# player4771/YOLO-DBL

Hardware: AMD Instinct MI355X
Metric: images/sec @640×640 bs=32 (1/2/4/8 GPU) + mAP@0.5 vs CPU ref (higher is better)
Workload: dtype fp16; 1 GPU; YOLO-DBL-n 640x640 bs=32/GPU fp16 forward+decode+NMS (conf .25, iou .7, max_det 300); model=yolov13n_DBL, global_batch=32, imgsz=640, nc=3, parallelism=dp1, streams_per_gpu=2

## Files before the change

include/ydbl.h:

```cpp
#ifndef YDBL_H
#define YDBL_H

#include <stdint.h>

#ifdef __cplusplus
extern "C" {
#endif

enum { YDBL_OK = 0, YDBL_EINVAL = 1, YDBL_ELAUNCH = 2, YDBL_ECAPACITY = 3 };
enum { YDBL_F32 = 0, YDBL_F16 = 1 };
enum { YDBL_ACT_NONE = 0, YDBL_ACT_SILU = 1, YDBL_ACT_GELU = 2, YDBL_ACT_SIGMOID = 3 };
enum { YDBL_RES_NONE = 0, YDBL_RES_ADD = 1, YDBL_RES_MUL = 2 };

typedef struct {
  void* ptr;
  int32_t n, h, w, c;
  int32_t cs;
  int32_t dtype;
} ydbl_view;

typedef struct {
  ydbl_view x, y, r;
  const void* w;
  const float* bias;
  int32_t kh, kw, stride, pad, dil;
  int32_t kpad;
  int32_t act, res_mode;
  ydbl_view y2, r2;
  float a2, b2;
  const float* dq;
  float qscale;
  void* workspace;
  int64_t workspace_bytes;
} ydbl_conv_desc;
int ydbl_conv2d_nhwc(const ydbl_conv_desc* d, void* stream);
int64_t ydbl_conv_workspace(const ydbl_conv_desc* d);

typedef struct {
  ydbl_view x, y, r;
  const float* dw_w;
  const void* pw_w;
  const float* bias;
  int32_t k, stride, pad, dil;
  int32_t kpad, act, res_mode;
  const float* dw_bias;
  int32_t dw_act;
  const float* tail_w;
  const float* tail_b;
  ydbl_view tail_y;
  int32_t tail_n;
  float* cand_box;
  float* cand_score;
  int32_t* cand_cls;
  int32_t* cand_idx;
  int32_t* cand_count;
  int32_t cand_cap;
  float conf_thres;
  int32_t multi_label;
  int32_t nclasses;
  const int32_t* classes;
  float level_stride;
  int32_t anchor0;
  ydbl_view box;
  int32_t zero_counts;
  int32_t y_unused;
  uint8_t* tile_mask;
  int32_t mask_tiles_x;
  int32_t mask_tiles_img;
  uint8_t* mask_zero;
  int32_t mask_zero_bytes;
} ydbl_dsconv_desc;
int ydbl_dsconv_nhwc(const ydbl_dsconv_desc* d, void* stream);

typedef struct {
  ydbl_view x, y, r;
  const float* w;
  const float* bias;
  int32_t kh, kw, stride, pad, dil;
  int32_t act, res_mode;
} ydbl_dwconv_desc;
int ydbl_dwconv2d_nhwc(const ydbl_dwconv_desc* d, void* stream);

int ydbl_dwconv2d_pair_nhwc(const ydbl_dwconv_desc* d0, const ydbl_dwconv_desc* d1, void* stream);

typedef struct {
  const float* const* x;
  const float* amax;
} ydbl_input_bind;

int32_t ydbl_batch_max_work_ints(void);
void ydbl_batch_max_work_init(int32_t* host_work);
int ydbl_batch_max(const float* x, int64_t n, int32_t* work, float* amax, float* scale, void* stream);
int ydbl_batch_max_bound(const float* const* xword, int64_t n, int32_t* work, float* amax, float* scale,
                         void* stream);

int ydbl_input_nchw_to_nhwc(const float* x, int32_t n, int32_t c, int32_t h, int32_t w, float scale,
                            const ydbl_view* y, const ydbl_input_bind* bind, void* stream);

int ydbl_conv_stem(const float* x, int32_t n, int32_t cin, int32_t h, int32_t w, float scale, const float* wt,
                   const float* bias, int32_t k, int32_t stride, int32_t act, const ydbl_view* y,
                   const ydbl_input_bind* bind, void* stream);

int ydbl_gate_add(const ydbl_view* a, const ydbl_view* b, float gate, const ydbl_view* y, void* stream);

int ydbl_channel_gate_add(const ydbl_view* a, const ydbl_view* b, const float* gate, const ydbl_view* y,
                          void* stream);

typedef struct {
  ydbl_view qkv, y, v;
  int32_t heads, area;
  float scale;
} ydbl_area_attn_desc;
int ydbl_area_attn(const ydbl_area_attn_desc* d, void* stream);

int ydbl_pool_up_concat(const ydbl_view* p_lo, const ydbl_view* p_mid, const ydbl_view* p_hi,
                        const ydbl_view* y, void* stream);

int ydbl_dysample(const ydbl_view* x, const ydbl_view* off, int32_t groups, const ydbl_view* y, void* stream);
typedef struct {
  ydbl_view x, off;
  int32_t groups;
  ydbl_view y, y2, r2;
  float a2, b2;
} ydbl_dysample_desc;
int ydbl_dysample_ex(const ydbl_dysample_desc* d, void* stream);
typedef struct {
  ydbl_view x;
  const void* off_w;
  const float* off_b;
  int32_t groups;
  ydbl_view y, y2, r2;
  float a2, b2;
} ydbl_dysample2_desc;
int ydbl_dysample2(const ydbl_dysample2_desc* d, void* stream);

int ydbl_lsk_gate(const ydbl_view* attn, const float* sw, const float* sb, const ydbl_view* out,
                  void* workspace, void* stream);
int64_t ydbl_lsk_gate_workspace(int32_t n, int32_t h, int32_t w);
typedef struct {
  ydbl_view x, a1, a2, attn, y;
  const void* w12;
  const float* b12;
  const float* sw;
  const float* sb;
  const void* w;
  const float* b;
  float* agg;
} ydbl_lsk_desc;
int ydbl_lsk_attn(const ydbl_lsk_desc* d, void* stream);
int ydbl_lsk_out(const ydbl_lsk_desc* d, void* stream);

typedef struct {
  ydbl_view x;
  ydbl_view xp;
  ydbl_view y;
  int32_t num_edges, num_heads;
  const float* proto_base;
  const float* ctx_w;
  const float* ctx_b;
  const float* edge_w;
  const float* edge_b;
  const float* node_w;
  const float* node_b;
  void* workspace;
  const void* pre_w;
  const float* pre_b;
} ydbl_hg_desc;
int64_t ydbl_hg_workspace(int32_t n, int32_t tokens, int32_t dim, int32_t edges);
int ydbl_hg_context(const ydbl_hg_desc* d, void* stream);
int ydbl_hg_propagate(const ydbl_hg_desc* d, void* stream);
int64_t ydbl_hg_fused_workspace(int32_t n, int32_t tokens, int32_t dim, int32_t edges, int32_t dtype);
int ydbl_hg_fused(const ydbl_hg_desc* d, void* stream);
int ydbl_hg_fused_pair(const ydbl_hg_desc* d0, const ydbl_hg_desc* d1, void* stream);

typedef struct {
  ydbl_view box[3], cls[3];
  int32_t nl, nc;
  float stride[3];
  float conf_thres;
  int32_t multi_label;
  const int32_t* classes; int32_t nclasses;
  float* y_ref;
  float* cand_box;
  float* cand_score;
  int32_t* cand_cls;
  int32_t* cand_idx;
  int32_t* cand_count;
  int32_t cap;
} ydbl_decode_desc;
int ydbl_detect_decode(const ydbl_decode_desc* d, void* stream);

typedef struct {
  float scale;
  float flip_w;
  int32_t a_lo, a_hi;
  int32_t pos_base;
  int32_t y_stride;
  int32_t append;
} ydbl_decode_aug;
int ydbl_detect_decode_aug(const ydbl_decode_desc* d, const ydbl_decode_aug* g, void* stream);

typedef struct {
  const float* pred;
  int32_t n, nc, A;
  float conf_thres;
  int32_t multi_label;
  const int32_t* classes; int32_t nclasses;
  float* cand_box; float* cand_score; int32_t* cand_cls; int32_t* cand_idx; int32_t* cand_count;
  int32_t cap;
} ydbl_pred_cand_desc;
int ydbl_pred_candidates(const ydbl_pred_cand_desc* d, void* stream);

typedef struct {
  const float* cand_box; const float* cand_score; const int32_t* cand_cls; const int32_t* cand_idx;
  const int32_t* cand_count;
  int32_t n, cap;
  double iou_thres;
  int32_t max_det, max_nms, agnostic;
  float max_wh;
  float clip_w, clip_h;
  float* out; int32_t* out_count;
  void* workspace;
  int64_t out_stride, count_stride;
  int32_t per_image;
} ydbl_nms_desc;
int64_t ydbl_nms_workspace(int32_t n, int32_t cap, int32_t max_nms);
int ydbl_nms(const ydbl_nms_desc* d, void* stream);

typedef struct {
  const float* x;
  int32_t n, cin, h, w;
  float scale;
  int32_t c0;
  const void* params;
  ydbl_view y;
  ydbl_input_bind bind;
// ... 163 lines not shown
```

yolo-dbl_amd/csrc/misc.hip:

```cpp
#include "common.hpp"

namespace ydbl {

template <typename T>
__global__ __launch_bounds__(256) void dwconv_kernel(DView<const T> x, DView<T> y, DView<const T> r,
                                                     const float* __restrict__ w, const float* __restrict__ bias,
                                                     int KH, int KW, int S, int PAD, int DIL, int act) {
  constexpr int V = Vec<T>::N;
  const int cg = y.c / V;
  const int64_t idx = (int64_t)blockIdx.x * blockDim.x + threadIdx.x;
  const int64_t total = (int64_t)y.n * y.h * y.w * cg;
  if (idx >= total) return;
  const int c0 = (int)(idx % cg) * V;
  int64_t pix = idx / cg;
  const int ox = (int)(pix % y.w);
  const int64_t t = pix / y.w;
  const int oy = (int)(t % y.h);
  const int b = (int)(t / y.h);
  float acc[V];
#pragma unroll
  for (int q = 0; q < V; ++q) acc[q] = 0.f;
  for (int ky = 0; ky < KH; ++ky) {
    const int iy = oy * S - PAD + ky * DIL;
    if (iy < 0 || iy >= x.h) continue;
// ... 331 lines not shown
    for (int q = 0; q < V; ++q) s[q] += v[q];
    load_f<V>(lo.at(b, 2 * oy + 1, 2 * ox) + c, v);
#pragma unroll
    for (int q = 0; q < V; ++q) s[q] += v[q];
    load_f<V>(lo.at(b, 2 * oy + 1, 2 * ox + 1) + c, v);
#pragma unroll
    for (int q = 0; q < V; ++q) o[q] = (s[q] + v[q]) / 4.0f;
  } else if (c < clo + cmid) {
    load_f<V>(mid.at(b, oy, ox) + (c - clo), o);
  } else {
    load_f<V>(hi.at(b, oy >> 1, ox >> 1) + (c - clo - cmid), o);
  }
  store_f<V>(y.at(b, oy, ox) + c, o);
}

template <typename T>
__global__ __launch_bounds__(256) void dysample_kernel(DView<const T> x, DView<const T> off, int G, DView<T> y,
                                                       DView<T> y2, DView<const T> r2, float a2, float b2) {
  constexpr int V = Vec<T>::N;
  const int cpg = x.c / G;
  const int cgv = cpg / V;
  const int64_t idx = (int64_t)blockIdx.x * blockDim.x + threadIdx.x;
  const int64_t total = (int64_t)y.n * y.h * y.w * G * cgv;
  if (idx >= total) return;
  const int cv = (int)(idx % cgv);
  int64_t t = idx / cgv;
  const int gi = (int)(t % G);
  t /= G;
  const int ox2 = (int)(t % y.w);
  t /= y.w;
  const int oy2 = (int)(t % y.h);
  const int b = (int)(t / y.h);
  const int H = x.h, W = x.w;
  const int h = oy2 >> 1, w = ox2 >> 1, si = oy2 & 1, sj = ox2 & 1;
  const T* op = off.at(b, h, w);
  const float offx = float(op[gi * 4 + si * 2 + sj]);
  const float offy = float(op[4 * G + gi * 4 + si * 2 + sj]);
  const float gx = 2.0f * ((float(w) + 0.5f) + offx) / float(W) - 1.0f;
  const float gy = 2.0f * ((float(h) + 0.5f) + offy) / float(H) - 1.0f;
  float ix = ((gx + 1.0f) * float(W) - 1.0f) / 2.0f;
  float iy = ((gy + 1.0f) * float(H) - 1.0f) / 2.0f;
  ix = fminf(float(W - 1), fmaxf(ix, 0.0f));
  iy = fminf(float(H - 1), fmaxf(iy, 0.0f));
  const int x0 = (int)floorf(ix), y0 = (int)floorf(iy);
  const int x1 = x0 + 1, y1 = y0 + 1;
  const float wnw = (float(x1) - ix) * (float(y1) - iy);
  const float wne = (ix - float(x0)) * (float(y1) - iy);
  const float wsw = (float(x1) - ix) * (iy - float(y0));
  const float wse = (ix - float(x0)) * (iy - float(y0));
  const int c0 = gi * cpg + cv * V;
  const bool xin = x1 < W, yin = y1 < H;
  const int x1c = xin ? x1 : x0, y1c = yin ? y1 : y0;
  float vnw[V], vne[V], vsw[V], vse[V];
  load_f<V>(x.at(b, y0, x0) + c0, vnw);
  load_f<V>(x.at(b, y0, x1c) + c0, vne);
  load_f<V>(x.at(b, y1c, x0) + c0, vsw);
  load_f<V>(x.at(b, y1c, x1c) + c0, vse);
  const float kne = xin ? wne : 0.f, ksw = yin ? wsw : 0.f, kse = xin && yin ? wse : 0.f;
  float acc[V];
#pragma unroll
  for (int q = 0; q < V; ++q) {
    acc[q] = blend4(vnw[q], wnw, vne[q], kne, vsw[q], ksw, vse[q], kse);
  }
  store_f<V>(y.at(b, oy2, ox2) + c0, acc);
  if (y2.p) {
    float rv[V], o2[V];
    load_f<V>(r2.at(b, oy2, ox2) + c0, rv);
#pragma unroll
    for (int q = 0; q < V; ++q) o2[q] = pad_mix(a2, round_to<T>(acc[q]), b2, rv[q]);
    store_f<V>(y2.at(b, oy2, ox2) + c0, o2);
  }
}

template <typename T>
__global__ __launch_bounds__(256) void lsk_stats_kernel(DView<const T> attn, float* __restrict__ agg) {
  constexpr int V = Vec<T>::N, L = 32;
  const int64_t t = (int64_t)blockIdx.x * blockDim.x + threadIdx.x;
  const int64_t pix = t / L;
  const int sub = (int)(t % L);
  const bool live = pix < (int64_t)attn.n * attn.h * attn.w;
  const T* p = attn.pix(live ? pix : 0);
  float s = 0.f, m = -INFINITY;
  for (int c = sub * V; c < attn.c; c += L * V) {
    float v[V];
    load_f<V>(p + c, v);
#pragma unroll
    for (int q = 0; q < V; ++q) {
      s += v[q];
      m = fmaxf(m, v[q]);
    }
  }
#pragma unroll
  for (int o = L / 2; o > 0; o >>= 1) {
    s += __shfl_xor(s, o);
    m = fmaxf(m, __shfl_xor(m, o));
  }
  if (live && sub == 0) {
    agg[pix * 2 + 0] = s / float(attn.c);
    agg[pix * 2 + 1] = m;
  }
}

template <typename T>
__global__ __launch_bounds__(256) void lsk_gate_kernel(DView<const T> attn, const float* __restrict__ agg,
                                                       const float* __restrict__ sw, const float* __restrict__ sb,
                                                       DView<T> out) {
  constexpr int V = Vec<T>::N;
  const int half = out.c;
  const int cg = half / V;
  const int64_t idx = (int64_t)blockIdx.x * blockDim.x + threadIdx.x;
  if (idx >= (int64_t)out.n * out.h * out.w * cg) return;
  const int c0 = (int)(idx % cg) * V;
  const int64_t pix = idx / cg;
  const int ox = (int)(pix % out.w);
  const int64_t t = pix / out.w;
  const int oy = (int)(t % out.h);
  const int b = (int)(t / out.h);
  const bool split = cg % 16 == 0;
  const int t0 = split ? (int)(idx & 15) : 0, ts = split ? 16 : 1;
  float s0 = 0.f, s1 = 0.f;
  for (int tap = t0; tap < 98; tap += ts) {
    const int ci = tap / 49, ky = (tap % 49) / 7, kx = tap % 7;
    const int iy = oy - 3 + ky, ix = ox - 3 + kx;
    if (iy < 0 || iy >= out.h || ix < 0 || ix >= out.w) continue;
    const float a = agg[(((int64_t)b * out.h + iy) * out.w + ix) * 2 + ci];
    s0 = fmaf(sw[((0 * 2 + ci) * 7 + ky) * 7 + kx], a, s0);
    s1 = fmaf(sw[((1 * 2 + ci) * 7 + ky) * 7 + kx], a, s1);
  }
  if (split) {
#pragma unroll
    for (int o = 8; o > 0; o >>= 1) {
      s0 += __shfl_xor(s0, o);
      s1 += __shfl_xor(s1, o);
    }
  }
  s0 = sigmoidf_(s0 + sb[0]);
  s1 = sigmoidf_(s1 + sb[1]);
  float a1[V], a2[V], o[V];
  load_f<V>(attn.pix(pix) + c0, a1);
  load_f<V>(attn.pix(pix) + half + c0, a2);
#pragma unroll
  for (int q = 0; q < V; ++q) o[q] = gate_mix(a1[q], s0, a2[q], s1);
  store_f<V>(out.pix(pix) + c0, o);
}

template <typename T>
static DView<const T> cview(const ydbl_view* v) {
  if (!v) return DView<const T>{nullptr, 0, 0, 0, 0, 0};
  return DView<const T>{reinterpret_cast<const T*>(v->ptr), v->n, v->h, v->w, v->c, v->cs};
}

static unsigned nblk(int64_t n) { return (unsigned)cdiv(n, 256); }

}

using namespace ydbl;

extern "C" int ydbl_dwconv2d_nhwc(const ydbl_dwconv_desc* d, void* stream) {
  if (!d) return fail(YDBL_EINVAL, "dwconv: null descriptor");
  if (check_view(&d->x, "dwconv.x", true) || check_view(&d->y, "dwconv.y", true)) return YDBL_EINVAL;
  if (d->x.c != d->y.c || d->x.n != d->y.n || d->x.dtype != d->y.dtype) return fail(YDBL_EINVAL, "dwconv: x/y mismatch");
  const int ho = (d->x.h + 2 * d->pad - d->dil * (d->kh - 1) - 1) / d->stride + 1;
  const int wo = (d->x.w + 2 * d->pad - d->dil * (d->kw - 1) - 1) / d->stride + 1;
  if (ho != d->y.h || wo != d->y.w) return fail(YDBL_EINVAL, "dwconv: output spatial size mismatch");
  if (!d->w) return fail(YDBL_EINVAL, "dwconv: null weights");
  const bool res = d->res_mode == YDBL_RES_ADD;
  if (d->res_mode != YDBL_RES_NONE && !res) return fail(YDBL_EINVAL, "dwconv: only residual ADD is supported");
  if (res && (check_view(&d->r, "dwconv.r", true) || d->r.c != d->y.c || d->r.n != d->y.n || d->r.h != d->y.h ||
              d->r.w != d->y.w || d->r.dtype != d->y.dtype))
    return fail(YDBL_EINVAL, "dwconv: residual shape mismatch");
  hipStream_t s = as_stream(stream);
  const int V = d->x.dtype == YDBL_F16 ? 8 : 4;
  const int64_t total = (int64_t)d->y.n * d->y.h * d->y.w * (d->y.c / V);
  if (d->kh == d->kw) {
    const bool done = d->x.dtype == YDBL_F16
                          ? launch_dw_lds<_Float16>(d, cview<_Float16>(&d->x), dview<_Float16>(d->y),
                                                   cview<_Float16>(res ? &d->r : nullptr), s)
                          : launch_dw_lds<float>(d, cview<float>(&d->x), dview<float>(d->y),
                                                cview<float>(res ? &d->r : nullptr), s);
    if (done) return check_launch("ydbl_dwconv2d_nhwc");
  }
  if (d->x.dtype == YDBL_F16)
    dwconv_kernel<_Float16><<<nblk(total), 256, 0, s>>>(cview<_Float16>(&d->x), dview<_Float16>(d->y),
                                                        cview<_Float16>(res ? &d->r : nullptr), d->w, d->bias,
                                                        d->kh, d->kw, d->stride, d->pad, d->dil, epi_act(d->act));
  else
    dwconv_kernel<float><<<nblk(total), 256, 0, s>>>(cview<float>(&d->x), dview<float>(d->y),
                                                     cview<float>(res ? &d->r : nullptr), d->w, d->bias, d->kh, d->kw,
                                                     d->stride, d->pad, d->dil, epi_act(d->act));
  return check_launch("ydbl_dwconv2d_nhwc");
}

extern "C" int ydbl_dwconv2d_pair_nhwc(const ydbl_dwconv_desc* d0, const ydbl_dwconv_desc* d1, void* stream) {
  if (!d0 || !d1) return fail(YDBL_EINVAL, "dw_pair: null descriptor");
  if (d1->x.ptr != d0->y.ptr || d1->x.cs != d0->y.cs || d1->x.c != d0->y.c)
    return fail(YDBL_EINVAL, "dw_pair: d1.x must be d0.y");
  const bool pair = d0->kh == 5 && d0->kw == 5 && d0->dil == 1 && d1->kh == 7 && d1->kw == 7 && d1->dil == 3 &&
                    d0->stride == 1 && d1->stride == 1 && d0->res_mode == YDBL_RES_NONE &&
                    d1->res_mode == YDBL_RES_NONE && d0->x.h == d0->y.h && d0->x.w == d0->y.w &&
                    d1->y.h == d0->y.h && d1->y.w == d0->y.w && d0->x.h * d0->x.w <= DWP_HWMAX &&
                    d0->x.dtype == d0->y.dtype && d1->y.dtype == d0->y.dtype && d0->x.c == d0->y.c &&
                    d1->y.c == d0->y.c && d0->x.n == d0->y.n && d1->y.n == d0->y.n;
  const int V = d0->x.dtype == YDBL_F16 ? 8 : 4;
  constexpr int CV = 2;
  if (!pair || d0->y.c % (CV * V) || !d0->w || !d1->w || check_view(&d0->x, "dw_pair.x", true) ||
      check_view(&d0->y, "dw_pair.y0", true) || check_view(&d1->y, "dw_pair.y1", true)) {
    const int r = ydbl_dwconv2d_nhwc(d0, stream);
    return r ? r : ydbl_dwconv2d_nhwc(d1, stream);
  }
  hipStream_t s = as_stream(stream);
  const unsigned blocks = (unsigned)(d0->y.n * (d0->y.c / (CV * V)));
  constexpr int NT = 1024;
  if (d0->x.dtype == YDBL_F16)
    dw_pair_kernel<_Float16, 5, 1, 7, 3, CV, NT><<<blocks, NT, 0, s>>>(
        cview<_Float16>(&d0->x), dview<_Float16>(d0->y), dview<_Float16>(d1->y), d0->w, d0->bias, d1->w, d1->bias,
        d0->pad, d1->pad, epi_act(d0->act), epi_act(d1->act));
  else
    dw_pair_kernel<float, 5, 1, 7, 3, CV, NT><<<blocks, NT, 0, s>>>(
        cview<float>(&d0->x), dview<float>(d0->y), dview<float>(d1->y), d0->w, d0->bias, d1->w, d1->bias, d0->pad,
        d1->pad, epi_act(d0->act), epi_act(d1->act));
  return check_launch("ydbl_dwconv2d_pair_nhwc");
}

extern "C" int ydbl_input_nchw_to_nhwc(const float* x, int32_t n, int32_t c, int32_t h, int32_t w, float scale,
                                       const ydbl_view* y, const ydbl_input_bind* bind, void* stream) {
  if (!x) return fail(YDBL_EINVAL, "input: null x");
  if (check_view(y, "input.y", true)) return YDBL_EINVAL;
  if (y->n != n || y->h != h || y->w != w || y->c < c) return fail(YDBL_EINVAL, "input: shape mismatch");
  hipStream_t s = as_stream(stream);
  const int64_t total = (int64_t)n * h * w;
  if (y->dtype == YDBL_F16)
    input_kernel<_Float16><<<nblk(total), 256, 0, s>>>(x, n, c, h, w, scale, dview<_Float16>(*y), input_bind(bind));
  else
    input_kernel<float><<<nblk(total), 256, 0, s>>>(x, n, c, h, w, scale, dview<float>(*y), input_bind(bind));
  return check_launch("ydbl_input_nchw_to_nhwc");
}

extern "C" int ydbl_gate_add(const ydbl_view* a, const ydbl_view* b, float gate, const ydbl_view* y, void* stream) {
  if (check_view(a, "gate.a", true) || check_view(b, "gate.b", true) || check_view(y, "gate.y", true)) return YDBL_EINVAL;
  if (a->c != y->c || b->c != y->c || a->n * a->h * a->w != y->n * y->h * y->w ||
      b->n * b->h * b->w != y->n * y->h * y->w || a->dtype != y->dtype || b->dtype != y->dtype)
    return fail(YDBL_EINVAL, "gate_add: shape mismatch");
  hipStream_t s = as_stream(stream);
  const int V = y->dtype == YDBL_F16 ? 8 : 4;
  const int64_t total = (int64_t)y->n * y->h * y->w * (y->c / V);
  if (y->dtype == YDBL_F16)
    gate_add_kernel<_Float16><<<nblk(total), 256, 0, s>>>(cview<_Float16>(a), cview<_Float16>(b), gate, dview<_Float16>(*y));
  else
    gate_add_kernel<float><<<nblk(total), 256, 0, s>>>(cview<float>(a), cview<float>(b), gate, dview<float>(*y));
  return check_launch("ydbl_gate_add");
}

extern "C" int ydbl_channel_gate_add(const ydbl_view* a, const ydbl_view* b, const float* gate, const ydbl_view* y,
                                     void* stream) {
  if (check_view(a, "cgate.a", true) || check_view(b, "cgate.b", true) || check_view(y, "cgate.y", true)) return YDBL_EINVAL;
  if (!gate || reinterpret_cast<uintptr_t>(gate) % 16) return fail(YDBL_EINVAL, "channel_gate_add: gate must be a 16-byte aligned fp32 vector");
  if (a->c != y->c || b->c != y->c || a->n * a->h * a->w != y->n * y->h * y->w ||
      b->n * b->h * b->w != y->n * y->h * y->w || a->dtype != y->dtype || b->dtype != y->dtype)
    return fail(YDBL_EINVAL, "channel_gate_add: shape mismatch");
  hipStream_t s = as_stream(stream);
  const int V = y->dtype == YDBL_F16 ? 8 : 4;
  const int64_t total = (int64_t)y->n * y->h * y->w * (y->c / V);
  if (y->dtype == YDBL_F16)
    channel_gate_add_kernel<_Float16><<<nblk(total), 256, 0, s>>>(cview<_Float16>(a), cview<_Float16>(b), gate,
                                                                   dview<_Float16>(*y));
  else
    channel_gate_add_kernel<float><<<nblk(total), 256, 0, s>>>(cview<float>(a), cview<float>(b), gate, dview<float>(*y));
  return check_launch("ydbl_channel_gate_add");
}

extern "C" int ydbl_pool_up_concat(const ydbl_view* lo, const ydbl_view* mid, const ydbl_view* hi, const ydbl_view* y,
                                   void* stream) {
  if (check_view(y, "concat.y", true)) return YDBL_EINVAL;
  int ctot = 0;
  if (lo) {
    if (check_view(lo, "concat.lo", true)) return YDBL_EINVAL;
    if (lo->h != 2 * y->h || lo->w != 2 * y->w || lo->n != y->n) return fail(YDBL_EINVAL, "concat: lo must be 2x output");
    ctot += lo->c;
  }
  if (mid) {
    if (check_view(mid, "concat.mid", true)) return YDBL_EINVAL;
    if (mid->h != y->h || mid->w != y->w || mid->n != y->n) return fail(YDBL_EINVAL, "concat: mid must match output");
    ctot += mid->c;
  }
  if (hi) {
    if (check_view(hi, "concat.hi", true)) return YDBL_EINVAL;
    if (2 * hi->h != y->h || 2 * hi->w != y->w || hi->n != y->n) return fail(YDBL_EINVAL, "concat: hi must be 1/2 output");
    ctot += hi->c;
  }
  if (ctot != y->c) return fail(YDBL_EINVAL, "concat: channel sum mismatch");
  hipStream_t s = as_stream(stream);
  const int V = y->dtype == YDBL_F16 ? 8 : 4;
  const int64_t total = (int64_t)y->n * y->h * y->w * (y->c / V);
  if (y->dtype == YDBL_F16)
    pool_up_concat_kernel<_Float16><<<nblk(total), 256, 0, s>>>(cview<_Float16>(lo), cview<_Float16>(mid),
                                                                 cview<_Float16>(hi), dview<_Float16>(*y));
  else
    pool_up_concat_kernel<float><<<nblk(total), 256, 0, s>>>(cview<float>(lo), cview<float>(mid), cview<float>(hi),
                                                              dview<float>(*y));
  return check_launch("ydbl_pool_up_concat");
}

static int dysample_go(const ydbl_view* x, const ydbl_view* off, int32_t groups, const ydbl_view* y,
                       const ydbl_view* y2, const ydbl_view* r2, float a2, float b2, void* stream) {
  if (check_view(x, "dysample.x", true) || check_view(off, "dysample.off", false) || check_view(y, "dysample.y", true))
    return YDBL_EINVAL;
  const int V = y->dtype == YDBL_F16 ? 8 : 4;
  if (groups < 1 || x->c % groups || (x->c / groups) % V) return fail(YDBL_EINVAL, "dysample: bad groups");
  if (off->c != 8 * groups || off->h != x->h || off->w != x->w || y->h != 2 * x->h || y->w != 2 * x->w ||
      y->c != x->c || off->dtype != x->dtype || y->dtype != x->dtype)
    return fail(YDBL_EINVAL, "dysample: shape mismatch");
  const bool two = y2 && y2->ptr;
  if (two) {
    if (check_view(y2, "dysample.y2", true) || check_view(r2, "dysample.r2", true)) return YDBL_EINVAL;
    auto same = [&](const ydbl_view* v) {
      return v->n == y->n && v->h == y->h && v->w == y->w && v->c == y->c && v->dtype == y->dtype;
    };
    if (!same(y2) || !same(r2)) return fail(YDBL_EINVAL, "dysample: y2/r2 must match y");
  }
  hipStream_t s = as_stream(stream);
  const int64_t total = (int64_t)y->n * y->h * y->w * groups * (x->c / groups / V);
  if (y->dtype == YDBL_F16)
    dysample_kernel<_Float16><<<nblk(total), 256, 0, s>>>(
        cview<_Float16>(x), cview<_Float16>(off), groups, dview<_Float16>(*y),
        two ? dview<_Float16>(*y2) : DView<_Float16>{nullptr, 0, 0, 0, 0, 0}, cview<_Float16>(two ? r2 : nullptr), a2, b2);
  else
    dysample_kernel<float><<<nblk(total), 256, 0, s>>>(
        cview<float>(x), cview<float>(off), groups, dview<float>(*y),
        two ? dview<float>(*y2) : DView<float>{nullptr, 0, 0, 0, 0, 0}, cview<float>(two ? r2 : nullptr), a2, b2);
  return check_launch("ydbl_dysample");
}

extern "C" int ydbl_dysample(const ydbl_view* x, const ydbl_view* off, int32_t groups, const ydbl_view* y,
                             void* stream) {
  return dysample_go(x, off, groups, y, nullptr, nullptr, 0.f, 0.f, stream);
}

extern "C" int ydbl_dysample_ex(const ydbl_dysample_desc* d, void* stream) {
  if (!d) return fail(YDBL_EINVAL, "dysample: null descriptor");
  return dysample_go(&d->x, &d->off, d->groups, &d->y, &d->y2, &d->r2, d->a2, d->b2, stream);
}

extern "C" int64_t ydbl_lsk_gate_workspace(int32_t n, int32_t h, int32_t w) { return (int64_t)n * h * w * 2 * 4; }

extern "C" int ydbl_lsk_gate(const ydbl_view* attn, const float* sw, const float* sb, const ydbl_view* out,
                             void* workspace, void* stream) {
  if (check_view(attn, "lsk.attn", true) || check_view(out, "lsk.out", true)) return YDBL_EINVAL;
  if (attn->c != 2 * out->c || attn->n != out->n || attn->h != out->h || attn->w != out->w ||
      attn->dtype != out->dtype)
    return fail(YDBL_EINVAL, "lsk: shape mismatch");
  if (!sw || !sb || !workspace) return fail(YDBL_EINVAL, "lsk: null weights/workspace");
  hipStream_t s = as_stream(stream);
  float* agg = reinterpret_cast<float*>(workspace);
  const int64_t npix = (int64_t)out->n * out->h * out->w;
  const int V = out->dtype == YDBL_F16 ? 8 : 4;
  if (out->dtype == YDBL_F16) {
    lsk_stats_kernel<_Float16><<<nblk(npix * 32), 256, 0, s>>>(cview<_Float16>(attn), agg);
    lsk_gate_kernel<_Float16><<<nblk(npix * (out->c / V)), 256, 0, s>>>(cview<_Float16>(attn), agg, sw, sb,
                                                                         dview<_Float16>(*out));
  } else {
    lsk_stats_kernel<float><<<nblk(npix * 32), 256, 0, s>>>(cview<float>(attn), agg);
    lsk_gate_kernel<float><<<nblk(npix * (out->c / V)), 256, 0, s>>>(cview<float>(attn), agg, sw, sb,
                                                                      dview<float>(*out));
// ... 4 lines not shown
```

yolo-dbl_amd/ydbl/_lib.py:

```python

from __future__ import annotations

import ctypes as C
import os
from pathlib import Path

import torch

LIB_PATH = Path(os.environ.get("YDBL_LIB", Path(__file__).resolve().parent / "libydbl.so"))

F32, F16 = 0, 1
ACT_NONE, ACT_SILU, ACT_GELU, ACT_SIGMOID = 0, 1, 2, 3
RES_NONE, RES_ADD, RES_MUL = 0, 1, 2


class View(C.Structure):
    _fields_ = [("ptr", C.c_void_p), ("n", C.c_int32), ("h", C.c_int32), ("w", C.c_int32), ("c", C.c_int32),
                ("cs", C.c_int32), ("dtype", C.c_int32)]


class ConvDesc(C.Structure):
    _fields_ = [("x", View), ("y", View), ("r", View), ("w", C.c_void_p), ("bias", C.c_void_p),
                ("kh", C.c_int32), ("kw", C.c_int32), ("stride", C.c_int32), ("pad", C.c_int32), ("dil", C.c_int32),
                ("kpad", C.c_int32), ("act", C.c_int32), ("res_mode", C.c_int32),
# ... 20 lines not shown
                ("zero_counts", C.c_int32), ("y_unused", C.c_int32),
                ("tile_mask", C.c_void_p), ("mask_tiles_x", C.c_int32), ("mask_tiles_img", C.c_int32),
                ("mask_zero", C.c_void_p), ("mask_zero_bytes", C.c_int32)]
    g2_w = g0_w = None


class HgDesc(C.Structure):
    _fields_ = [("x", View), ("xp", View), ("y", View), ("num_edges", C.c_int32), ("num_heads", C.c_int32),
                ("proto_base", C.c_void_p), ("ctx_w", C.c_void_p), ("ctx_b", C.c_void_p),
                ("edge_w", C.c_void_p), ("edge_b", C.c_void_p), ("node_w", C.c_void_p), ("node_b", C.c_void_p),
                ("workspace", C.c_void_p), ("pre_w", C.c_void_p), ("pre_b", C.c_void_p)]


class DecodeDesc(C.Structure):
    _fields_ = [("box", View * 3), ("cls", View * 3), ("nl", C.c_int32), ("nc", C.c_int32),
                ("stride", C.c_float * 3), ("conf_thres", C.c_float), ("multi_label", C.c_int32),
                ("classes", C.c_void_p), ("nclasses", C.c_int32), ("y_ref", C.c_void_p),
                ("cand_box", C.c_void_p), ("cand_score", C.c_void_p), ("cand_cls", C.c_void_p),
                ("cand_idx", C.c_void_p), ("cand_count", C.c_void_p), ("cap", C.c_int32)]


class DecodeAug(C.Structure):
    _fields_ = [("scale", C.c_float), ("flip_w", C.c_float), ("a_lo", C.c_int32), ("a_hi", C.c_int32),
                ("pos_base", C.c_int32), ("y_stride", C.c_int32), ("append", C.c_int32)]


class ScaleImgDesc(C.Structure):
    _fields_ = [("x", C.c_void_p), ("n", C.c_int32), ("c", C.c_int32), ("h", C.c_int32), ("w", C.c_int32),
                ("sh", C.c_int32), ("sw", C.c_int32), ("hp", C.c_int32), ("wp", C.c_int32), ("flip", C.c_int32),
                ("pad_value", C.c_float), ("y", C.c_void_p)]


class PredCandDesc(C.Structure):
    _fields_ = [("pred", C.c_void_p), ("n", C.c_int32), ("nc", C.c_int32), ("A", C.c_int32),
                ("conf_thres", C.c_float), ("multi_label", C.c_int32), ("classes", C.c_void_p),
                ("nclasses", C.c_int32), ("cand_box", C.c_void_p), ("cand_score", C.c_void_p),
                ("cand_cls", C.c_void_p), ("cand_idx", C.c_void_p), ("cand_count", C.c_void_p), ("cap", C.c_int32)]


class NmsDesc(C.Structure):
    _fields_ = [("cand_box", C.c_void_p), ("cand_score", C.c_void_p), ("cand_cls", C.c_void_p),
                ("cand_idx", C.c_void_p), ("cand_count", C.c_void_p), ("n", C.c_int32), ("cap", C.c_int32),
                ("iou_thres", C.c_double), ("max_det", C.c_int32), ("max_nms", C.c_int32), ("agnostic", C.c_int32),
                ("max_wh", C.c_float), ("clip_w", C.c_float), ("clip_h", C.c_float), ("out", C.c_void_p),
                ("out_count", C.c_void_p), ("workspace", C.c_void_p), ("out_stride", C.c_int64),
                ("count_stride", C.c_int64), ("per_image", C.c_int32)]


class InputBind(C.Structure):
    _fields_ = [("x", C.c_void_p), ("amax", C.c_void_p)]


class Stem2Desc(C.Structure):
    _fields_ = [("x", C.c_void_p), ("n", C.c_int32), ("cin", C.c_int32), ("h", C.c_int32), ("w", C.c_int32),
                ("scale", C.c_float), ("c0", C.c_int32), ("params", C.c_void_p), ("y", View), ("bind", InputBind)]


class DySampleDesc(C.Structure):
    _fields_ = [("x", View), ("off", View), ("groups", C.c_int32), ("y", View), ("y2", View), ("r2", View),
                ("a2", C.c_float), ("b2", C.c_float)]


class DySample2Desc(C.Structure):
    _fields_ = [("x", View), ("off_w", C.c_void_p), ("off_b", C.c_void_p), ("groups", C.c_int32), ("y", View),
                ("y2", View), ("r2", View), ("a2", C.c_float), ("b2", C.c_float)]


class LskDesc(C.Structure):
    _fields_ = [("x", View), ("a1", View), ("a2", View), ("attn", View), ("y", View), ("w12", C.c_void_p),
                ("b12", C.c_void_p), ("sw", C.c_void_p), ("sb", C.c_void_p), ("w", C.c_void_p), ("b", C.c_void_p),
                ("agg", C.c_void_p)]


class BottleneckDesc(C.Structure):
    _fields_ = [("x", View), ("y", View), ("c", C.c_int32), ("add", C.c_int32), ("tile_h", C.c_int32),
                ("params", C.c_void_p), ("c_mid", C.c_int32), ("pw", C.c_int32),
                ("tile_mask", C.c_void_p), ("cand_box", C.c_void_p), ("cand_idx", C.c_void_p),
                ("cand_count", C.c_void_p), ("cand_cap", C.c_int32), ("level_stride", C.c_float),
                ("anchor0", C.c_int32), ("nc", C.c_int32), ("multi_label", C.c_int32)]


class LetterboxDesc(C.Structure):
    _fields_ = [("src", C.c_void_p), ("src_off", C.c_void_p), ("meta", C.c_void_p), ("n", C.c_int32),
                ("out_h", C.c_int32), ("out_w", C.c_int32), ("pad_value", C.c_float), ("out", C.c_void_p)]


class MatchDesc(C.Structure):
    _fields_ = [("det", C.c_void_p), ("det_count", C.c_void_p), ("n", C.c_int32), ("max_det", C.c_int32),
                ("gt_box", C.c_void_p), ("gt_cls", C.c_void_p), ("gt_ofs", C.c_void_p), ("n_gt", C.c_int32),
                ("iouv", C.c_void_p), ("n_iou", C.c_int32), ("single_cls", C.c_int32), ("correct", C.c_void_p),
                ("workspace", C.c_void_p)]


class ConfusionDesc(C.Structure):
    _fields_ = [("det", C.c_void_p), ("det_count", C.c_void_p), ("n", C.c_int32), ("max_det", C.c_int32),
                ("gt_box", C.c_void_p), ("gt_cls", C.c_void_p), ("gt_ofs", C.c_void_p), ("n_gt", C.c_int32),
                ("nc", C.c_int32), ("conf", C.c_float), ("iou_thres", C.c_float), ("matrix", C.c_void_p),
                ("invalid", C.c_void_p), ("workspace", C.c_void_p)]


class CocoDesc(C.Structure):
    _fields_ = [("det", C.c_void_p), ("det_count", C.c_void_p), ("n", C.c_int32), ("max_det", C.c_int32),
                ("gt_box", C.c_void_p), ("gt_cls", C.c_void_p), ("gt_ofs", C.c_void_p), ("n_gt", C.c_int32),
                ("single_cls", C.c_int32), ("nc", C.c_int32), ("iou_thrs", C.c_void_p), ("n_iou", C.c_int32),
                ("area_rng", C.c_void_p), ("n_area", C.c_int32), ("max_dets", C.c_int32), ("dt_rank", C.c_void_p),
                ("dt_matched", C.c_void_p), ("dt_ignored", C.c_void_p), ("gt_ignore", C.c_void_p),
                ("invalid", C.c_void_p), ("workspace", C.c_void_p)]


class AreaAttnDesc(C.Structure):
    _fields_ = [("qkv", View), ("y", View), ("v", View), ("heads", C.c_int32), ("area", C.c_int32),
                ("scale", C.c_float)]


class AvgPoolDesc(C.Structure):
    _fields_ = [("x", View), ("y", C.c_void_p), ("y_stride", C.c_int64), ("workspace", C.c_void_p),
                ("workspace_bytes", C.c_int64)]


class TrackDesc(C.Structure):
    _fields_ = [("det", C.c_void_p), ("det_count", C.c_void_p), ("n", C.c_int32), ("max_det", C.c_int32),
                ("det_stride", C.c_int64), ("count_stride", C.c_int64), ("hw", C.c_void_p),
                ("track_high_thresh", C.c_double), ("track_low_thresh", C.c_double),
                ("new_track_thresh", C.c_double), ("match_thresh", C.c_double), ("fuse_score", C.c_int32),
                ("track_buffer", C.c_int32), ("max_time_lost", C.c_int32), ("max_tracks", C.c_int32),
                ("trackers", C.c_int32), ("reset_each", C.c_int32), ("out", C.c_void_p), ("out_count", C.c_void_p),
                ("tracked", C.c_void_p), ("out_idx", C.c_void_p), ("state", C.c_void_p), ("state_bytes", C.c_int64)]


class LossDesc(C.Structure):
    _fields_ = [("box", View * 3), ("cls", View * 3), ("nl", C.c_int32), ("nc", C.c_int32), ("reg_max", C.c_int32),
                ("stride", C.c_float * 3), ("gt", C.c_void_p), ("max_labels", C.c_int32), ("topk", C.c_int32),
                ("gain_box", C.c_float), ("gain_cls", C.c_float), ("gain_dfl", C.c_float),
                ("loss", C.c_void_p), ("target_scores_sum", C.c_void_p), ("per_image", C.c_void_p),
                ("fg", C.c_void_p), ("target_gt_idx", C.c_void_p), ("target_score", C.c_void_p),
                ("workspace", C.c_void_p), ("workspace_bytes", C.c_int64)]


class LossGradDesc(C.Structure):
    _fields_ = [("box", View * 3), ("cls", View * 3), ("nl", C.c_int32), ("nc", C.c_int32), ("reg_max", C.c_int32),
                ("stride", C.c_float * 3), ("gt", C.c_void_p), ("max_labels", C.c_int32),
                ("gain_box", C.c_float), ("gain_cls", C.c_float), ("gain_dfl", C.c_float),
                ("fg", C.c_void_p), ("target_gt_idx", C.c_void_p), ("target_score", C.c_void_p),
                ("target_scores_sum", C.c_void_p), ("grad_scale", C.c_void_p), ("batch_scale", C.c_float),
                ("gbox", View * 3), ("gcls", View * 3)]


_P = C.c_void_p
_VP = C.POINTER(View)
SIGNATURES = {
    "ydbl_conv2d_nhwc": ([C.POINTER(ConvDesc), _P], C.c_int),
    "ydbl_dwconv2d_nhwc": ([C.POINTER(DwConvDesc), _P], C.c_int),
    "ydbl_dwconv2d_pair_nhwc": ([C.POINTER(DwConvDesc), C.POINTER(DwConvDesc), _P], C.c_int),
    "ydbl_dsconv_nhwc": ([C.POINTER(DsConvDesc), _P], C.c_int),
    "ydbl_batch_max_work_ints": ([], C.c_int32),
    "ydbl_batch_max_work_init": ([_P], None),
    "ydbl_batch_max": ([_P, C.c_int64, _P, _P, _P, _P], C.c_int),
    "ydbl_batch_max_bound": ([_P, C.c_int64, _P, _P, _P, _P], C.c_int),
    "ydbl_input_nchw_to_nhwc": ([_P, C.c_int32, C.c_int32, C.c_int32, C.c_int32, C.c_float, _VP,
                                 C.POINTER(InputBind), _P], C.c_int),
    "ydbl_conv_stem": ([_P, C.c_int32, C.c_int32, C.c_int32, C.c_int32, C.c_float, _P, _P, C.c_int32, C.c_int32,
                        C.c_int32, _VP, C.POINTER(InputBind), _P], C.c_int),
    "ydbl_gate_add": ([_VP, _VP, C.c_float, _VP, _P], C.c_int),
    "ydbl_channel_gate_add": ([_VP, _VP, _P, _VP, _P], C.c_int),
    "ydbl_area_attn": ([C.POINTER(AreaAttnDesc), _P], C.c_int),
    "ydbl_pool_up_concat": ([_VP, _VP, _VP, _VP, _P], C.c_int),
    "ydbl_dysample": ([_VP, _VP, C.c_int32, _VP, _P], C.c_int),
    "ydbl_dysample_ex": ([C.POINTER(DySampleDesc), _P], C.c_int),
    "ydbl_lsk_gate": ([_VP, _P, _P, _VP, _P, _P], C.c_int),
    "ydbl_lsk_gate_workspace": ([C.c_int32, C.c_int32, C.c_int32], C.c_int64),
    "ydbl_lsk_attn": ([C.POINTER(LskDesc), _P], C.c_int),
    "ydbl_lsk_out": ([C.POINTER(LskDesc), _P], C.c_int),
    "ydbl_hg_workspace": ([C.c_int32, C.c_int32, C.c_int32, C.c_int32], C.c_int64),
    "ydbl_hg_context": ([C.POINTER(HgDesc), _P], C.c_int),
    "ydbl_hg_propagate": ([C.POINTER(HgDesc), _P], C.c_int),
    "ydbl_hg_fused_workspace": ([C.c_int32, C.c_int32, C.c_int32, C.c_int32, C.c_int32], C.c_int64),
    "ydbl_hg_fused": ([C.POINTER(HgDesc), _P], C.c_int),
    "ydbl_hg_fused_pair": ([C.POINTER(HgDesc), C.POINTER(HgDesc), _P], C.c_int),
    "ydbl_dysample2": ([C.POINTER(DySample2Desc), _P], C.c_int),
    "ydbl_detect_decode": ([C.POINTER(DecodeDesc), _P], C.c_int),
    "ydbl_detect_decode_aug": ([C.POINTER(DecodeDesc), C.POINTER(DecodeAug), _P], C.c_int),
    "ydbl_scale_img": ([C.POINTER(ScaleImgDesc), _P], C.c_int),
    "ydbl_pred_candidates": ([C.POINTER(PredCandDesc), _P], C.c_int),
    "ydbl_nms_workspace": ([C.c_int32, C.c_int32, C.c_int32], C.c_int64),
    "ydbl_conv_workspace": ([C.POINTER(ConvDesc)], C.c_int64),
    "ydbl_nms": ([C.POINTER(NmsDesc), _P], C.c_int),
    "ydbl_conv_stem2_params_size": ([C.c_int32], C.c_int64),
    "ydbl_conv_stem2_pack": ([_P, _P, _P, _P, C.c_int32, _P], C.c_int),
    "ydbl_conv_stem2": ([C.POINTER(Stem2Desc), _P], C.c_int),
    "ydbl_bottleneck_params_size": ([C.c_int32], C.c_int64),
    "ydbl_bottleneck_pack": ([_P, _P, _P, _P, C.c_int32, _P], C.c_int),
    "ydbl_bottleneck_nhwc": ([C.POINTER(BottleneckDesc), _P], C.c_int),
    "ydbl_conv3x3_pair_params_size": ([C.c_int32, C.c_int32], C.c_int64),
    "ydbl_conv3x3_pair_pack": ([_P, _P, _P, _P, C.c_int32, C.c_int32, _P], C.c_int),
    "ydbl_detect_box_params_size": ([C.c_int32, C.c_int32], C.c_int64),
    "ydbl_detect_box_pack": ([_P, _P, _P, _P, _P, _P, C.c_int32, C.c_int32, _P], C.c_int),
    "ydbl_letterbox": ([C.POINTER(LetterboxDesc), _P], C.c_int),
    "ydbl_match_workspace": ([C.c_int32, C.c_int32, C.c_int32, C.c_int32], C.c_int64),
    "ydbl_match_predictions": ([C.POINTER(MatchDesc), _P], C.c_int),
    "ydbl_confusion_workspace": ([C.c_int32, C.c_int32, C.c_int32], C.c_int64),
    "ydbl_confusion_matrix": ([C.POINTER(ConfusionDesc), _P], C.c_int),
    "ydbl_coco_workspace": ([C.c_int32, C.c_int32, C.c_int32, C.c_int32], C.c_int64),
    "ydbl_coco_match": ([C.POINTER(CocoDesc), _P], C.c_int),
    "ydbl_global_avgpool_workspace": ([C.POINTER(AvgPoolDesc)], C.c_int64),
    "ydbl_global_avgpool": ([C.POINTER(AvgPoolDesc), _P], C.c_int),
    "ydbl_bytetrack_state_bytes": ([C.c_int32, C.c_int32], C.c_int64),
    "ydbl_bytetrack_update": ([C.POINTER(TrackDesc), _P], C.c_int),
    "ydbl_detect_loss_workspace": ([C.c_int32, C.c_int32, C.c_int32], C.c_int64),
    "ydbl_detect_loss": ([C.POINTER(LossDesc), _P], C.c_int),
    "ydbl_detect_loss_grad": ([C.POINTER(LossGradDesc), _P], C.c_int),
    "ydbl_last_error": ([], C.c_char_p),
    "ydbl_version": ([], C.c_char_p),
}


def _load():
    if not LIB_PATH.exists():
        raise ImportError(
            f"libydbl.so not found at {LIB_PATH}; build it with `python -c \"import __graft_entry__ as g; g.build()\"` "
            "(the HIP path has no fallback)"
        )
    lib = C.CDLL(str(LIB_PATH))
    for name, (args, res) in SIGNATURES.items():
        fn = getattr(lib, name)
        fn.argtypes = args
        fn.restype = res
    return lib


lib = _load()


class YdblError(RuntimeError):
    pass


def check(rc: int, what: str = ""):
    if rc != 0:
        msg = lib.ydbl_last_error().decode(errors="replace")
        raise YdblError(f"{what or 'ydbl'} failed (code {rc}): {msg}")


def dtype_code(dt: torch.dtype) -> int:
    if dt == torch.float16:
        return F16
    if dt == torch.float32:
        return F32
    raise TypeError(f"unsupported activation dtype {dt}")


def version() -> str:
    return lib.ydbl_version().decode()


def batch_max_work(device) -> "torch.Tensor":
    import torch

    host = torch.empty(int(lib.ydbl_batch_max_work_ints()), dtype=torch.int32)
    lib.ydbl_batch_max_work_init(host.data_ptr())
    return host.to(device)
```

yolo-dbl_amd/ydbl/runtime.py:

```python

from __future__ import annotations

import ctypes as C
import operator
import os
import time
from dataclasses import dataclass, field

import torch

from . import _lib
from ._lib import View, lib


SWITCHES = ("YDBL_DS2_OFF", "YDBL_DS_LEAN", "YDBL_HG_UNFUSED", "YDBL_HALO_NB", "YDBL_HALO_SMALL", "YDBL_VW", "YDBL_WSK_HALF",
            "YDBL_LSK_FUSE", "YDBL_NMS_FAST", "YDBL_NMS_GROUPS", "YDBL_SPLITK", "YDBL_NO_BNECK", "YDBL_NO_BOX3",
            "YDBL_NO_CLS_TAIL", "YDBL_DWPW", "YDBL_NO_PAIR3", "YDBL_NO_FUSE_PAD", "YDBL_NO_MERGE", "YDBL_NO_STEM2",
            "YDBL_EPI_GENERIC", "YDBL_NO_SPARSE_BOX", "YDBL_NO_HG_PAIR")


def ydbl_env() -> tuple:
    get = os.environ.get
    return tuple(get(k) for k in SWITCHES)


_STRUCT_EPOCH = [0]


def _bump_epoch(*_):
    _STRUCT_EPOCH[0] += 1


for _reg in ("register_module_parameter_registration_hook", "register_module_buffer_registration_hook",
             "register_module_module_registration_hook"):
    getattr(torch.nn.modules.module, _reg)(_bump_epoch)
_VERSION = operator.attrgetter("_version")


def weights_signature(module: torch.nn.Module) -> tuple:
    c = module.__dict__.get("_wsig_cache")
    if c is None or c[0] != _STRUCT_EPOCH[0]:
        ts = [t for t in (*module.parameters(), *module.buffers()) if t.is_floating_point()]
        c = (_STRUCT_EPOCH[0], ts, hash(tuple((id(t), t.data_ptr()) for t in ts)))
        module.__dict__["_wsig_cache"] = c
    return c[2], sum(map(_VERSION, c[1]))


def round_up(x: int, m: int) -> int:
    return (x + m - 1) // m * m


class TV:

    __slots__ = ("base", "off", "n", "h", "w", "c", "cs")

    def __init__(self, base: torch.Tensor, off: int, n: int, h: int, w: int, c: int, cs: int):
        self.base, self.off, self.n, self.h, self.w, self.c, self.cs = base, off, n, h, w, c, cs

    @property
    def dtype(self):
        return self.base.dtype

    @property
    def ptr(self) -> int:
        return self.base.data_ptr() + self.off * self.base.element_size()

    @property
    def shape(self):
        return (self.n, self.h, self.w, self.c)

    def cslice(self, c0: int, c: int) -> "TV":
        assert 0 <= c0 and c0 + c <= self.c, (c0, c, self.c)
        return TV(self.base, self.off + c0, self.n, self.h, self.w, c, self.cs)

    def with_hw(self, h: int, w: int) -> "TV":
        assert h * w == self.h * self.w
        return TV(self.base, self.off, self.n, h, w, self.c, self.cs)

    def struct(self) -> View:
        return View(self.ptr, self.n, self.h, self.w, self.c, self.cs, _lib.dtype_code(self.dtype))

    def torch(self) -> torch.Tensor:
        return torch.as_strided(
            self.base, (self.n, self.h, self.w, self.c), (self.h * self.w * self.cs, self.w * self.cs, self.cs, 1),
            self.off,
        )

    def nchw(self) -> torch.Tensor:
        return self.torch().permute(0, 3, 1, 2)


@dataclass
class Step:
    fn: object
    args: tuple
    what: str
    keep: list = field(default_factory=list)


class Plan:

    def __init__(self, device: torch.device, dtype: torch.dtype):
        self.device = torch.device(device)
        self.dtype = dtype
        self.steps: list[Step] = []
        self.buffers: list[torch.Tensor] = []
        self.bytes_allocated = 0
        self._writers: dict = {}
        self.fp8_candidates: list = []
        self.fp8_layers: list = []

    def alloc(self, n: int, h: int, w: int, c: int, dtype: torch.dtype | None = None, cs: int | None = None) -> TV:
        dtype = dtype or self.dtype
        cs = cs or round_up(c, 8)
        t = torch.empty(n * h * w * cs, dtype=dtype, device=self.device)
        self.buffers.append(t)
        self.bytes_allocated += t.numel() * t.element_size()
        return TV(t, 0, n, h, w, c, cs)

    def scratch(self, nbytes: int, zero: bool = False) -> torch.Tensor:
        t = (torch.zeros if zero else torch.empty)(max(int(nbytes), 16), dtype=torch.uint8, device=self.device)
        self.buffers.append(t)
        self.bytes_allocated += t.numel()
        return t

    def splitk_scratch(self, nbytes: int) -> torch.Tensor:
        cur = getattr(self, "_splitk", None)
        if cur is None or cur.numel() < nbytes:
            cur = self._splitk = self.scratch(nbytes)
        return cur

    def const(self, t: torch.Tensor) -> torch.Tensor:
        t = t.detach().to(self.device).contiguous()
        self.buffers.append(t)
        return t

    def launch(self, name: str, *args, what: str = "", keep=()):
        self.steps.append(Step(getattr(lib, name), args, what or name, list(keep)))

    @staticmethod
    def _vkey(v: TV):
        return (v.base.data_ptr(), v.off, v.n, v.h, v.w, v.c, v.cs)

    def note_writer(self, y: TV, desc) -> None:
        self._writers[self._vkey(y)] = (len(self.steps) - 1, desc)

    def writer_of(self, v: TV):
        return self._writers.get(self._vkey(v))

    def made_before(self, v: TV, step: int) -> bool:
        w = self.writer_of(v)
        return w is not None and w[0] < step

    def fuse_second_output(self, writer, y2: TV, r2: TV, a2: float, b2: float) -> TV | None:
        _, d = writer
        if not hasattr(d, "y2") or d.y2.ptr:
            return None
        y = d.y
        for v in (y2, r2):
            if (v.n, v.h, v.w, v.c) != (y.n, y.h, y.w, y.c) or _lib.dtype_code(v.dtype) != y.dtype or v.cs % 4:
                return None
            if isinstance(d, (_lib.DySampleDesc, _lib.DySample2Desc)):
                vec = 16 // v.base.element_size()
                if v.cs % vec or v.c % vec or v.ptr % 16:
                    return None
        d.y2, d.r2, d.a2, d.b2 = y2.struct(), r2.struct(), float(a2), float(b2)
        self.steps[writer[0]].keep.append((y2, r2))
        return y2

    def check_single_stream(self):
        for st in self.steps:
# ... 131 lines not shown
```

Before: 18850 images/s.

## Add fast fused 5x5+dilated 7x7 depthwise pair kernel with LDS-staged padded tiles

Adds a specialised fp16 kernel for the LSK-style depthwise pair (5x5 then 7x7 dilation 3) on small feature maps. Each block stages two channel groups of the whole padded input in LDS, computes the first conv and writes its output both to global memory and into a zero-padded LDS buffer, then computes the dilated conv from LDS. It uses v_fma_mix with scalar weights loaded through constant address space, so there is no f16-to-f32 unpack step and boundary checks are removed. A routing function picks this path when the shapes fit and the old kernel is not forced by an environment switch, at the cost of high LDS use per block.

```diff
diff --git a/include/ydbl.h b/include/ydbl.h
--- a/include/ydbl.h
+++ b/include/ydbl.h
@@ -82,6 +82,7 @@
 int ydbl_dwconv2d_nhwc(const ydbl_dwconv_desc* d, void* stream);
 
 int ydbl_dwconv2d_pair_nhwc(const ydbl_dwconv_desc* d0, const ydbl_dwconv_desc* d1, void* stream);
+int ydbl_dwconv2d_pair_route(const ydbl_dwconv_desc* d0, const ydbl_dwconv_desc* d1);
 
 typedef struct {
   const float* const* x;
diff --git a/yolo-dbl_amd/csrc/dw_pair.hip b/yolo-dbl_amd/csrc/dw_pair.hip
--- /dev/null
+++ b/yolo-dbl_amd/csrc/dw_pair.hip
@@ -0,0 +1,141 @@
+#include "common.hpp"
+
+namespace ydbl {
+
+constexpr int DWF_CV = 2;
+constexpr int DWF_NT = 1024;
+constexpr int DWF_HWMAX = 512;
+constexpr int DWF_LDS_MAX = 80 * 1024;
+
+template <int HI>
+__device__ __forceinline__ float fma_mix(uint32_t x, float w, float acc) {
+  if constexpr (HI)
+    asm("v_fma_mix_f32 %0, %1, %2, %0 op_sel:[1,0,0] op_sel_hi:[1,0,0]" : "+v"(acc) : "v"(x), "s"(w));
+  else
+    asm("v_fma_mix_f32 %0, %1, %2, %0 op_sel:[0,0,0] op_sel_hi:[1,0,0]" : "+v"(acc) : "v"(x), "s"(w));
+  return acc;
+}
+
+using u32x4 = __attribute__((ext_vector_type(4))) uint32_t;
+using cfp = const __attribute__((address_space(4))) float*;
+
+template <int K, int D>
+__device__ __forceinline__ void dwf_taps(const u32x4* src, int PW, const float* __restrict__ wg, int C, float* acc) {
+  const cfp w = (cfp)wg;
+#pragma unroll
+  for (int ky = 0; ky < K; ++ky) {
+    const u32x4* row = src + ky * D * PW;
+    float wr[K][8];
+    u32x4 xr[K];
+#pragma unroll
+    for (int kx = 0; kx < K; ++kx) {
+      xr[kx] = row[kx * D];
+#pragma unroll
+      for (int q = 0; q < 8; ++q) wr[kx][q] = w[(ky * K + kx) * C + q];
+    }
+    __builtin_amdgcn_sched_barrier(0);
+#pragma unroll
+    for (int kx = 0; kx < K; ++kx)
+#pragma unroll
+      for (int h = 0; h < 4; ++h) {
+        acc[2 * h] = fma_mix<0>(xr[kx][h], wr[kx][2 * h], acc[2 * h]);
+        acc[2 * h + 1] = fma_mix<1>(xr[kx][h], wr[kx][2 * h + 1], acc[2 * h + 1]);
+      }
+    __builtin_amdgcn_sched_barrier(0);
+  }
+}
+
+__global__ __launch_bounds__(DWF_NT) void dw_pair_fast_kernel(DView<const _Float16> x, DView<_Float16> y0,
+                                                               DView<_Float16> y1, const float* __restrict__ w0,
+                                                               const float* __restrict__ b0,
+                                                               const float* __restrict__ w1,
+                                                               const float* __restrict__ b1) {
+  constexpr int V = 8, CV = DWF_CV, P0 = 2, P1 = 9;
+  extern __shared__ __align__(16) unsigned char dwf_lds[];
+  const int C = y0.c, H = x.h, W = x.w, HW = H * W;
+  const int PW0 = W + 2 * P0, PH0 = H + 2 * P0, PW1 = W + 2 * P1, PH1 = H + 2 * P1;
+  const int N0 = PH0 * PW0, N1 = PH1 * PW1;
+  u32x4* sx = reinterpret_cast<u32x4*>(dwf_lds);
+  u32x4* sa = sx + CV * N0;
+  const int cgroups = C / (CV * V);
+  const int bid = xcd_remap(blockIdx.x, gridDim.x);
+  const int b = bid / cgroups, c0 = (bid % cgroups) * CV * V;
+  const int tid = threadIdx.x;
+  for (int i = tid; i < CV * N0; i += DWF_NT) {
+    const int cv = i % CV, pp = i / CV;
+    const int yy = pp / PW0 - P0, xx = pp % PW0 - P0;
+    const bool ok = yy >= 0 && yy < H && xx >= 0 && xx < W;
+    const h8 v = vload_sel(x.at(b, ok ? yy : 0, ok ? xx : 0) + c0 + cv * V, x.p, ok);
+    sx[cv * N0 + pp] = __builtin_bit_cast(u32x4, v);
+  }
+  for (int i = tid; i < CV * N1; i += DWF_NT) {
+    const int cv = i / N1, pp = i % N1;
+    const int yy = pp / PW1 - P1, xx = pp % PW1 - P1;
+    if (!(yy >= 0 && yy < H && xx >= 0 && xx < W)) sa[cv * N1 + pp] = u32x4{0u, 0u, 0u, 0u};
+  }
+  __syncthreads();
+  const int wave = wave_id();
+  const int cv = wave / (DWF_NT / 64 / CV);
+  const int p = (wave % (DWF_NT / 64 / CV)) * 64 + (tid & 63);
+  const int cc = c0 + cv * V;
+  const bool live = p < HW;
+  const int oy = live ? p / W : 0, ox = live ? p % W : 0;
+
+  float acc[V];
+#pragma unroll
+  for (int q = 0; q < V; ++q) acc[q] = 0.f;
+  dwf_taps<5, 1>(sx + cv * N0 + oy * PW0 + ox, PW0, w0 + cc, C, acc);
+  if (b0) {
+#pragma unroll
+    for (int q = 0; q < V; ++q) acc[q] += b0[cc + q];
+  }
+  {
+    h8 o;
+#pragma unroll
+    for (int q = 0; q < V; ++q) o[q] = f16_rne(acc[q]);
+    if (live) {
+      vstore(y0.at(b, oy, ox) + cc, o);
+      sa[cv * N1 + (oy + P1) * PW1 + ox + P1] = __builtin_bit_cast(u32x4, o);
+    }
+  }
+  __syncthreads();
+#pragma unroll
+  for (int q = 0; q < V; ++q) acc[q] = 0.f;
+  dwf_taps<7, 3>(sa + cv * N1 + oy * PW1 + ox, PW1, w1 + cc, C, acc);
+  if (b1) {
+#pragma unroll
+    for (int q = 0; q < V; ++q) acc[q] += b1[cc + q];
+  }
+  if (live) {
+    h8 o;
+#pragma unroll
+    for (int q = 0; q < V; ++q) o[q] = f16_rne(acc[q]);
+    vstore(y1.at(b, oy, ox) + cc, o);
+  }
+}
+
+static int64_t dwf_lds_bytes(int H, int W) {
+  return (int64_t)DWF_CV * 16 * ((int64_t)(H + 4) * (W + 4) + (int64_t)(H + 18) * (W + 18));
+}
+
+bool dw_pair_fast_ok(const ydbl_dwconv_desc* d0, const ydbl_dwconv_desc* d1) {
+  const char* e = getenv("YDBL_DW_PAIR_OLD");
+  if (e && *e == '1') return false;
+  return d0->x.dtype == YDBL_F16 && d0->act == YDBL_ACT_NONE && d1->act == YDBL_ACT_NONE && d0->pad == 2 &&
+         d1->pad == 9 && d0->x.h * d0->x.w <= DWF_HWMAX && dwf_lds_bytes(d0->x.h, d0->x.w) <= DWF_LDS_MAX &&
+         !epi_generic();
+}
+
+int dw_pair_fast_launch(const ydbl_dwconv_desc* d0, const ydbl_dwconv_desc* d1, hipStream_t s) {
+  static const hipError_t attr = hipFuncSetAttribute(reinterpret_cast<const void*>(dw_pair_fast_kernel),
+                                                     hipFuncAttributeMaxDynamicSharedMemorySize, DWF_LDS_MAX);
+  if (attr != hipSuccess) return fail(YDBL_ELAUNCH, std::string("dw_pair: ") + hipGetErrorString(attr));
+  const unsigned blocks = (unsigned)(d0->y.n * (d0->y.c / (DWF_CV * 8)));
+  const DView<const _Float16> xv{reinterpret_cast<const _Float16*>(d0->x.ptr), d0->x.n, d0->x.h, d0->x.w, d0->x.c,
+                                 d0->x.cs};
+  dw_pair_fast_kernel<<<blocks, DWF_NT, (size_t)dwf_lds_bytes(d0->x.h, d0->x.w), s>>>(
+      xv, dview<_Float16>(d0->y), dview<_Float16>(d1->y), d0->w, d0->bias, d1->w, d1->bias);
+  return check_launch("ydbl_dwconv2d_pair_nhwc");
+}
+
+}
diff --git a/yolo-dbl_amd/csrc/misc.hip b/yolo-dbl_amd/csrc/misc.hip
--- a/yolo-dbl_amd/csrc/misc.hip
+++ b/yolo-dbl_amd/csrc/misc.hip
@@ -507,6 +507,9 @@
 
 static unsigned nblk(int64_t n) { return (unsigned)cdiv(n, 256); }
 
+bool dw_pair_fast_ok(const ydbl_dwconv_desc* d0, const ydbl_dwconv_desc* d1);
+int dw_pair_fast_launch(const ydbl_dwconv_desc* d0, const ydbl_dwconv_desc* d1, hipStream_t s);
+
 }
 
 using namespace ydbl;
@@ -546,10 +549,8 @@
   return check_launch("ydbl_dwconv2d_nhwc");
 }
 
-extern "C" int ydbl_dwconv2d_pair_nhwc(const ydbl_dwconv_desc* d0, const ydbl_dwconv_desc* d1, void* stream) {
-  if (!d0 || !d1) return fail(YDBL_EINVAL, "dw_pair: null descriptor");
-  if (d1->x.ptr != d0->y.ptr || d1->x.cs != d0->y.cs || d1->x.c != d0->y.c)
-    return fail(YDBL_EINVAL, "dw_pair: d1.x must be d0.y");
+constexpr int DWP_CV = 2;
+static int dw_pair_route(const ydbl_dwconv_desc* d0, const ydbl_dwconv_desc* d1) {
   const bool pair = d0->kh == 5 && d0->kw == 5 && d0->dil == 1 && d1->kh == 7 && d1->kw == 7 && d1->dil == 3 &&
                     d0->stride == 1 && d1->stride == 1 && d0->res_mode == YDBL_RES_NONE &&
                     d1->res_mode == YDBL_RES_NONE && d0->x.h == d0->y.h && d0->x.w == d0->y.w &&
@@ -557,13 +558,30 @@
                     d0->x.dtype == d0->y.dtype && d1->y.dtype == d0->y.dtype && d0->x.c == d0->y.c &&
                     d1->y.c == d0->y.c && d0->x.n == d0->y.n && d1->y.n == d0->y.n;
   const int V = d0->x.dtype == YDBL_F16 ? 8 : 4;
-  constexpr int CV = 2;
-  if (!pair || d0->y.c % (CV * V) || !d0->w || !d1->w || check_view(&d0->x, "dw_pair.x", true) ||
-      check_view(&d0->y, "dw_pair.y0", true) || check_view(&d1->y, "dw_pair.y1", true)) {
+  if (!pair || d0->y.c % (DWP_CV * V) || !d0->w || !d1->w || check_view(&d0->x, "dw_pair.x", true) ||
+      check_view(&d0->y, "dw_pair.y0", true) || check_view(&d1->y, "dw_pair.y1", true))
+    return 0;
+  return dw_pair_fast_ok(d0, d1) ? 2 : 1;
+}
+
+extern "C" int ydbl_dwconv2d_pair_route(const ydbl_dwconv_desc* d0, const ydbl_dwconv_desc* d1) {
+  if (!d0 || !d1) return -1;
+  return dw_pair_route(d0, d1);
+}
+
+extern "C" int ydbl_dwconv2d_pair_nhwc(const ydbl_dwconv_desc* d0, const ydbl_dwconv_desc* d1, void* stream) {
+  if (!d0 || !d1) return fail(YDBL_EINVAL, "dw_pair: null descriptor");
+  if (d1->x.ptr != d0->y.ptr || d1->x.cs != d0->y.cs || d1->x.c != d0->y.c)
+    return fail(YDBL_EINVAL, "dw_pair: d1.x must be d0.y");
+  const int route = dw_pair_route(d0, d1);
+  if (route == 0) {
     const int r = ydbl_dwconv2d_nhwc(d0, stream);
     return r ? r : ydbl_dwconv2d_nhwc(d1, stream);
   }
   hipStream_t s = as_stream(stream);
+  if (route == 2) return dw_pair_fast_launch(d0, d1, s);
+  constexpr int CV = DWP_CV;
+  const int V = d0->x.dtype == YDBL_F16 ? 8 : 4;
   const unsigned blocks = (unsigned)(d0->y.n * (d0->y.c / (CV * V)));
   constexpr int NT = 1024;
   if (d0->x.dtype == YDBL_F16)
diff --git a/yolo-dbl_amd/ydbl/_lib.py b/yolo-dbl_amd/ydbl/_lib.py
--- a/yolo-dbl_amd/ydbl/_lib.py
+++ b/yolo-dbl_amd/ydbl/_lib.py
@@ -196,6 +196,7 @@
     "ydbl_conv2d_nhwc": ([C.POINTER(ConvDesc), _P], C.c_int),
     "ydbl_dwconv2d_nhwc": ([C.POINTER(DwConvDesc), _P], C.c_int),
     "ydbl_dwconv2d_pair_nhwc": ([C.POINTER(DwConvDesc), C.POINTER(DwConvDesc), _P], C.c_int),
+    "ydbl_dwconv2d_pair_route": ([C.POINTER(DwConvDesc), C.POINTER(DwConvDesc)], C.c_int),
     "ydbl_dsconv_nhwc": ([C.POINTER(DsConvDesc), _P], C.c_int),
     "ydbl_batch_max_work_ints": ([], C.c_int32),
     "ydbl_batch_max_work_init": ([_P], None),
diff --git a/yolo-dbl_amd/ydbl/runtime.py b/yolo-dbl_amd/ydbl/runtime.py
--- a/yolo-dbl_amd/ydbl/runtime.py
+++ b/yolo-dbl_amd/ydbl/runtime.py
@@ -16,7 +16,7 @@
 SWITCHES = ("YDBL_DS2_OFF", "YDBL_DS_LEAN", "YDBL_HG_UNFUSED", "YDBL_HALO_NB", "YDBL_HALO_SMALL", "YDBL_VW", "YDBL_WSK_HALF",
             "YDBL_LSK_FUSE", "YDBL_NMS_FAST", "YDBL_NMS_GROUPS", "YDBL_SPLITK", "YDBL_NO_BNECK", "YDBL_NO_BOX3",
             "YDBL_NO_CLS_TAIL", "YDBL_DWPW", "YDBL_NO_PAIR3", "YDBL_NO_FUSE_PAD", "YDBL_NO_MERGE", "YDBL_NO_STEM2",
-            "YDBL_EPI_GENERIC", "YDBL_NO_SPARSE_BOX", "YDBL_NO_HG_PAIR")
+            "YDBL_EPI_GENERIC", "YDBL_NO_SPARSE_BOX", "YDBL_NO_HG_PAIR", "YDBL_DW_PAIR_OLD")
 
 
 def ydbl_env() -> tuple:
```

Measured after the change: 19050 images/s (median of 6 runs). 1.1% higher.
